# hpc4cmb/flacarray

Measured on AMD Instinct MI355X. Metric: Msamples/s encode+decode, 4096ch x 1Msamp int32, higher is better.
Workload: dtype int32

## Files before the change

### flacarray_amd/csrc/encode_fused.hpp

```cpp
#pragma once
#include "encode_kernels.hpp"
#include "quantize_kernels.hpp"

namespace fa {

constexpr int kFSmpWords = 65 * 32;
#ifndef FA_F_SCANW
#define FA_F_SCANW 4
#endif
#ifndef FA_F_RING
#define FA_F_RING 1024
#endif
constexpr int kFRingWords = FA_F_RING;
constexpr int kFRingMask = kFRingWords - 1;
constexpr int kFRingBlocks = kFRingWords / 64;
constexpr int kFRowBlocks = 12;
static_assert(kFRingBlocks - kFRowBlocks - 1 >= 1, "the ring must hold the longest row and a partial block beside what waits to be flushed");
constexpr int kFWaveWords = kFSmpWords + kFRingWords + 4 + 16;
constexpr int kFWaves = 4;
constexpr int kFCrcSlice = 1024;
constexpr int kFCrcXpow = 520;
#ifndef FA_F_SLEEP
#define FA_F_SLEEP 8
#endif
#ifndef FA_F_WBATCH
#define FA_F_WBATCH 4
#endif
#ifndef FA_F_CEIL
#define FA_F_CEIL 1
#endif
#ifndef FA_F_BFLY_N
#define FA_F_BFLY_N 1
#endif
#ifndef FA_F_SHLEV
#define FA_F_SHLEV 1
#endif
#ifndef FA_F_SHLEV_MAXMLO
#define FA_F_SHLEV_MAXMLO 12
#endif
#ifndef FA_F_SHPOLL
#define FA_F_SHPOLL 256
#endif
#ifndef FA_F_SHSLEEP
#define FA_F_SHSLEEP 4
#endif
#ifndef FA_F_PARKN
#define FA_F_PARKN 32
#endif
#ifndef FA_F_PARKBLK
#define FA_F_PARKBLK 1
#endif
#ifndef FA_F_PARK
#define FA_F_PARK 1
#endif
#ifndef FA_F_WAVES
#define FA_F_WAVES 3
#endif
constexpr uint32_t kLbSpinLimit = 1u << 22;

struct FusedArgs {
    const int32_t* data;
    const float* f_offsets;
    const float* f_gains;
    int64_t n_stream, stream_size, nframes, total_frames;
    int32_t max_lpc_order, max_porder, precision, pmax_full;
    int32_t tail_bs;
    double escale_full;
    const float* win;
    const uint4* hdr;
    uint8_t* blob;
    int64_t capacity;
    int64_t hb;
    uint32_t* frame_bytes;
    int64_t* frame_abs;
    FrameInfo* info;
    uint32_t* ticket;
    uint32_t* size_pub;
    unsigned long long* off_pub;
    int64_t* total;
    int* err;
    const uint16_t* crc_tab;
    unsigned long long* stamps;
    int64_t* starts;
    int64_t* nbytes;
};

__device__ __forceinline__ int fsmp_unit(int c1, int u) { return 32 * c1 + 4 * (u ^ (c1 & 7)); }
__device__ __forceinline__ int fsmp_idx(int s) {
    const int c1 = (s >> 5) + 1;
    return fsmp_unit(c1, (s >> 2) & 7) + (s & 3);
}

__device__ __forceinline__ int lane_id_opaque() {
    int l;
    asm volatile("v_mbcnt_lo_u32_b32 %0, -1, 0\n\tv_mbcnt_hi_u32_b32 %0, -1, %0" : "=v"(l));
    return l;
}
__device__ __forceinline__ int rice_fold(int r) { return (int)(((uint32_t)r << 1) ^ (uint32_t)(r >> 31)); }
__device__ __forceinline__ int dpp_wave_shr1(int old, int v) { return __builtin_amdgcn_update_dpp(old, v, 0x138, 0xF, 0xF, false); }

__device__ __forceinline__ uint16_t crc16_mulmod(uint16_t a, uint16_t b) {
    uint32_t r = 0;
#pragma unroll
    for (int i = 15; i >= 0; --i) {
        r = (r << 1) ^ ((r & 0x8000u) ? 0x18005u : 0u);
        if ((b >> i) & 1) r ^= a;
    }
    return (uint16_t)r;
}

template <typename T>
__device__ __forceinline__ T lb_load(const T* p) { return __hip_atomic_load(p, __ATOMIC_RELAXED, __HIP_MEMORY_SCOPE_AGENT); }

struct SplitRiceSearch {
    int pred_order, pmax, lane;
    uint32_t TA, TB, S, n, pb, SC, best;
    int M, p, k, bpo, kb;
    bool slot;
    __device__ __forceinline__ void start(uint32_t ta, uint32_t tb, int pred_order_, int pmax_, int lane_) {
        pred_order = pred_order_; pmax = pmax_; lane = lane_;
        TA = wave_incl_scan_u32(ta);
        TB = wave_incl_scan_u32(tb);
    }
    __device__ __forceinline__ void gather() {
        M = (2 << pmax) - 1;
        const int Lp = M - lane;
        slot = (Lp >= 1);
        const int po = slot ? (31 - __clz(Lp)) : 0;
        p = lane - (M + 1 - (2 << po));
        const uint32_t psz = 4096u >> po;
        const int cpp = 128 >> po;
        const bool inB = (po > 0) && (p >= (1 << (po - 1)));
        const int ph = inB ? (p - (1 << (po - 1))) : p;
        int hi_l = (po == 0) ? 63 : ((ph + 1) * cpp - 1);
        int lo_l = (po == 0) ? -1 : (ph * cpp - 1);
        hi_l &= 63;
        const int lo_c = lo_l < 0 ? 0 : (lo_l & 63);
        const uint32_t ah = (uint32_t)__builtin_amdgcn_ds_bpermute(hi_l << 2, (int)TA);
        const uint32_t bh = (uint32_t)__builtin_amdgcn_ds_bpermute(hi_l << 2, (int)TB);
        const uint32_t al = (uint32_t)__builtin_amdgcn_ds_bpermute(lo_c << 2, (int)TA);
        const uint32_t bl = (uint32_t)__builtin_amdgcn_ds_bpermute(lo_c << 2, (int)TB);
        uint32_t s;
        if (po == 0) s = ah + bh;
        else s = (inB ? bh : ah) - ((lo_l >= 0) ? (inB ? bl : al) : 0u);
        S = slot ? s : 0u;
        n = psz - ((p == 0) ? (uint32_t)pred_order : 0u);
        n = slot ? n : 1u;
    }
    __device__ __forceinline__ void params() {
        const uint32_t fpd = 0x40000u / n;
        const uint32_t m1 = S - 1;
        const uint32_t v = (__umulhi(m1, fpd) << 14) | ((m1 * fpd) >> 18);
        k = (S < 2 || v == 0) ? 0 : (32 - __clz((int)v));
        const uint32_t rest = (k != 0) ? (S >> ((k - 1) & 31)) : (S << 1);
        pb = 4u + (uint32_t)(1 + k) * n + rest - (n >> 1);
        pb = slot ? pb : 0u;
    }
    __device__ __forceinline__ void totals() {
        SC = wave_incl_scan_u32(pb);
        best = 0xffffffffu;
        bpo = 0;
        kb = 0;
    }
    __device__ __forceinline__ void order(int o) {
        const bool valid = (o <= pmax);
        const int base = valid ? (M + 1 - (2 << o)) : 0;
        const int end = valid ? (base + (1 << o) - 1) : 0;
        const uint32_t hi = (uint32_t)__builtin_amdgcn_readlane((int)SC, end);
        const uint32_t lo = (uint32_t)__builtin_amdgcn_readlane((int)SC, base > 0 ? base - 1 : 0);
        const uint32_t bits = hi - (base > 0 ? lo : 0u) + 6u;
        const int kg = __builtin_amdgcn_ds_bpermute(((base + lane) & 63) << 2, k);
        const bool take = valid && (bits < best);
        best = take ? bits : best;
        bpo = take ? o : bpo;
        kb = take ? kg : kb;
    }
};

__device__ __forceinline__ uint64_t split_rice_search_slow(uint64_t ta, uint64_t tb, int pred_order, int pmax, int lane, int* best_po,
                                                           int* kbest) {
    const uint64_t TA = wave_incl_scan_u64(ta), TB = wave_incl_scan_u64(tb);
    uint64_t best = 0;
    bool have = false;
    int bpo = 0, kb = 0;
    for (int po = pmax; po >= 0; --po) {
        const int nparts = 1 << po;
        const uint32_t psz = 4096u >> po;
        const int cpp = 128 >> po;
        const int p = lane & (nparts - 1);
        const bool inB = (po > 0) && (p >= (nparts >> 1));
        const int ph = inB ? (p - (nparts >> 1)) : p;
        const int hi_l = (po == 0) ? 63 : (((ph + 1) * cpp - 1) & 63);
        const int lo_l = (po == 0) ? -1 : (ph * cpp - 1);
        const int lo_c = lo_l < 0 ? 0 : (lo_l & 63);
        const uint64_t ah = gather_u64(TA, hi_l), bh = gather_u64(TB, hi_l), al = gather_u64(TA, lo_c), bl = gather_u64(TB, lo_c);
        uint64_t S;
        if (po == 0) S = ah + bh;
        else S = (inB ? bh : ah) - ((lo_l >= 0) ? (inB ? bl : al) : 0);
        uint64_t pb = 0;
        int k = 0;
        if (lane < nparts) {
            const uint32_t n = psz - ((lane == 0) ? (uint32_t)pred_order : 0u);
            k = rice_param(S, n);
// ... 142 lines not shown
                for (int o = 0; o < MLO; ++o) {
                    const double b = mbv[o];
                    if (o < usable && b < bestb) { bestb = b; bi = o; }
                }
            }
            wlo = bi + 1;
        }
        if (fbps <= 17) {
            const int limp = 32 - fbps - ilog2_u64((uint64_t)wlo);
            if (wprec > limp) wprec = limp;
        }
        wsh = 0;
#pragma unroll
        for (int j = 0; j < MLO; ++j) wq[j] = 0;
        wok = 0;
        if (wprec >= 2) wok = (quantize_coefs_t<MLO>(coef + (wlo - 1) * MLO, wlo, wprec, wq, &wsh) == 0) ? 1 : 0;
    };
    auto shlev_announce = [&](bool cand, int fbps, const double* ac) __attribute__((always_inline)) {
        const int ln = lane_id_opaque();
        if (ln == 0) {
            if (cand) {
#pragma unroll
                for (int j = 0; j <= MLO; ++j) lev_in[wave][j] = ac[j];
            }
            lev_bps[wave] = cand ? fbps : -1;
        }
        lds_fence();
        uint32_t before = 0;
        if (ln == 0) before = __hip_atomic_fetch_add(&lev_cnt, 1u, __ATOMIC_RELAXED, __HIP_MEMORY_SCOPE_WORKGROUP);
        lds_fence();
        if ((uint32_t)__builtin_amdgcn_readfirstlane((int)before) != (uint32_t)(kFWaves - 1)) return;
        const int fr = ln >> 4, sub = ln & 15;
        const int fbps_w = lev_bps[fr];
        double acw[MLO + 1];
#pragma unroll
        for (int j = 0; j <= MLO; ++j) acw[j] = lev_in[fr][j];
        if (fbps_w < 0) {
            acw[0] = 1.0;
#pragma unroll
            for (int j = 1; j <= MLO; ++j) acw[j] = 0.0;
        }
        int wok, wlo, wprec, wsh;
        int32_t wq[MLO];
        lpc_solve(std::integral_constant<int, 16>{}, acw, fbps_w, scr + 256 * fr, sub, wok, wlo, wprec, wsh, wq);
        if (sub == 0) {
            lev_out[fr][0] = wok; lev_out[fr][1] = wlo; lev_out[fr][2] = wprec; lev_out[fr][3] = wsh;
#pragma unroll
            for (int j = 0; j < MLO; ++j) lev_out[fr][4 + j] = wq[j];
        }
        lds_fence();
        if (sub == 0) __hip_atomic_store(&lev_rdy[fr], 1u, __ATOMIC_RELAXED, __HIP_MEMORY_SCOPE_WORKGROUP);
        lds_fence();
    };
    if constexpr (SHLEV) {
        bool mine = g < a.total_frames;
        if (mine && a.tail_bs != kMaxBlock) mine = ((uint32_t)g % (uint32_t)a.nframes) != (uint32_t)(a.nframes - 1);
        if (__builtin_expect(!mine, 0)) {
            shlev_announce(false, 0, nullptr);
            return;
        }
    }
    if (g >= a.total_frames) return;

    const int64_t s = (int64_t)((uint32_t)g / (uint32_t)a.nframes);
    const int64_t f = g - s * a.nframes;
    if (f == a.nframes - 1 && a.tail_bs != kMaxBlock) return;
    const int32_t* src = a.data + (s * a.stream_size + f * (int64_t)bs);
    float q_off = 0.0f, q_gain = 0.0f;
    if constexpr (F32IN) { q_off = a.f_offsets[s]; q_gain = a.f_gains[s]; }
    auto load_row = [&](int j) __attribute__((always_inline)) {
        const int4 v = reinterpret_cast<const int4*>(src)[64 * j + lane];
        if constexpr (F32IN)
            return make_int4(quantise_f32(__int_as_float(v.x), q_off, q_gain), quantise_f32(__int_as_float(v.y), q_off, q_gain),
                             quantise_f32(__int_as_float(v.z), q_off, q_gain), quantise_f32(__int_as_float(v.w), q_off, q_gain));
        else
            return v;
    };
    const float* win = a.win;
    const uint4 fhe = a.hdr[f];
    const uint32_t fh_bits = 32u + ((fhe.w >> 8) & 0xFFu) + ((fhe.w >> 16) & 0xFFu) + (fhe.w >> 24) + 8u;

#define FA_IMAGE_ADDRS                                                                  \
    const int ln_ = lane_id_opaque();                                                   \
    const int K = fsmp_unit(ln_ + 1, 0);                                                \
    const int rowbase = fsmp_unit((ln_ >> 3) + 1, ln_ & 7);                             \
    const int hist7 = fsmp_unit(ln_, 7), hist6 = fsmp_unit(ln_, 6), hist5 = fsmp_unit(ln_, 5); \
    (void)K; (void)rowbase; (void)hist7; (void)hist6; (void)hist5
    constexpr int tailA7 = 32 * 64 + 4 * (7 ^ (64 & 7)), tailA6 = 32 * 64 + 4 * (6 ^ (64 & 7)), tailA5 = 32 * 64 + 4 * (5 ^ (64 & 7));

    FA_STAMP_INIT;
#ifdef FA_TIMELINE
    const uint32_t tl_start_ = (uint32_t)__builtin_amdgcn_s_memrealtime();
#endif
    int4 Bv[8];
    uint32_t orv = 0;
    int mn, mx;
    {
        FA_IMAGE_ADDRS;
        int4 hi[8], lo[8];
#pragma unroll
        for (int j = 0; j < 8; ++j) hi[j] = load_row(8 + j);
#pragma unroll
        for (int j = 0; j < 8; ++j) lo[j] = load_row(j);
        if (lane < 32) smp[lane] = 0;
        mn = hi[0].x;
        mx = hi[0].x;
#pragma unroll
        for (int j = 0; j < 8; ++j) {
            orv |= (uint32_t)(hi[j].x | hi[j].y | hi[j].z | hi[j].w);
            mn = min(min(mn, hi[j].x), hi[j].y);
            mn = min(min(mn, hi[j].z), hi[j].w);
            mx = max(max(mx, hi[j].x), hi[j].y);
            mx = max(max(mx, hi[j].z), hi[j].w);
            *reinterpret_cast<int4*>(&smp[rowbase + 256 * j]) = hi[j];
        }
#pragma unroll
        for (int t = 0; t < 8; ++t) Bv[t] = *reinterpret_cast<const int4*>(&smp[K ^ (4 * t)]);
#pragma unroll
        for (int j = 0; j < 8; ++j) {
// ... 129 lines not shown
#pragma unroll
            for (int t = 0; t < 4; ++t) group(std::false_type{}, Bv[t], 0);
            fold();
#pragma unroll
            for (int t = 4; t < 8; ++t) group(std::false_type{}, Bv[t], 0);
            fold();
            tot0 = (double)a0; tot1 = (double)a1; tot2 = (double)a2; tot3 = (double)a3; tot4 = (double)a4;
        } else {
            FA_IMAGE_ADDRS;
            double p1, pe1, pe2, pe3;
            auto seed = [&](const int4& h) __attribute__((always_inline)) {
                p1 = (double)h.w;
                pe1 = (double)h.w - (double)h.z;
                const double e1b = (double)h.z - (double)h.y;
                pe2 = pe1 - e1b;
                const double e2b = e1b - ((double)h.y - (double)h.x);
                pe3 = pe2 - e2b;
            };
            auto group = [&](const int4& xv, int gi0) __attribute__((always_inline)) {
                const int xs[4] = {xv.x, xv.y, xv.z, xv.w};
#pragma unroll
                for (int e = 0; e < 4; ++e) {
                    const int gi = gi0 + e;
                    const double xd = (double)xs[e];
                    const double e1 = xd - p1;
                    const double e2 = e1 - pe1;
                    const double e3 = e2 - pe2;
                    const double e4 = e3 - pe3;
                    const double a0 = fa_fabs(xd);
                    const double a1 = (gi >= 1) ? fa_fabs(e1) : 0.0;
                    const double a2 = (gi >= 2) ? fa_fabs(e2) : 0.0;
                    const double a3 = (gi >= 3) ? fa_fabs(e3) : 0.0;
                    const double a4 = (gi >= 4) ? fa_fabs(e4) : 0.0;
                    tot0 += a0; tot1 += a1; tot2 += a2; tot3 += a3; tot4 += a4;
                    mx0 = __builtin_fmax(mx0, a0);
                    mx1 = __builtin_fmax(mx1, a1);
                    mx2 = __builtin_fmax(mx2, a2);
                    mx3 = __builtin_fmax(mx3, a3);
                    mx4 = __builtin_fmax(mx4, a4);
                    p1 = xd; pe1 = e1; pe2 = e2; pe3 = e3;
                }
            };
            seed(*reinterpret_cast<const int4*>(&smp[hist7]));
#pragma unroll 1
            for (int t = 0; t < 8; ++t) group(*reinterpret_cast<const int4*>(&smp[K ^ (4 * t)]), 32 * lane + 4 * t);
            dA0 = tot0; dA1 = tot1; dA2 = tot2; dA3 = tot3; dA4 = tot4;
            seed(hist_b(Bv[7], *reinterpret_cast<const int4*>(&smp[tailA7])));
#pragma unroll
            for (int t = 0; t < 8; ++t) group(Bv[t], 4096);
        }
        FA_STAMP(1);
        {
            double tsum[5] = {tot0, tot1, tot2, tot3, tot4};
            wave_sum_butterfly_n<5>(tsum);
            const double T0 = tsum[0], T1 = tsum[1], T2 = tsum[2], T3 = tsum[3], T4 = tsum[4];
            double M0 = 0.0, M1 = 0.0, M2 = 0.0, M3 = 0.0, M4 = 0.0;
            if (!narrow) {
                M0 = wave_max_f64(mx0); M1 = wave_max_f64(mx1); M2 = wave_max_f64(mx2); M3 = wave_max_f64(mx3);
                M4 = wave_max_f64(mx4);
            }
            const double lim = 2147483647.0;
            double smallest = 1.8446744073709552e19;
            if (M0 <= lim && T0 < smallest) { fo = 0; smallest = T0; }
            if (M1 <= lim && T1 < smallest) { fo = 1; smallest = T1; }
            if (M2 <= lim && T2 < smallest) { fo = 2; smallest = T2; }
            if (M3 <= lim && T3 < smallest) { fo = 3; smallest = T3; }
            if (M4 <= lim && T4 < smallest) { fo = 4; smallest = T4; }
        }
        if (narrow) {
            const uint64_t tA = (fo == 0) ? hA0 : (fo == 1) ? hA1 : (fo == 2) ? hA2 : (fo == 3) ? hA3 : hA4;
            const double tt = (fo == 0) ? tot0 : (fo == 1) ? tot1 : (fo == 2) ? tot2 : (fo == 3) ? tot3 : tot4;
            fixA = tA;
            fixB = (uint64_t)tt - tA;
        } else {
            const double tA = (fo == 0) ? dA0 : (fo == 1) ? dA1 : (fo == 2) ? dA2 : (fo == 3) ? dA3 : dA4;
            const double tt = (fo == 0) ? tot0 : (fo == 1) ? tot1 : (fo == 2) ? tot2 : (fo == 3) ? tot3 : tot4;
            fixA = (uint64_t)tA;
            fixB = (uint64_t)(tt - tA);
        }
        pmax_fix = pmax_for(fo < 0 ? 0 : fo);
        const bool small_fix = __all((fixA < (1u << 24)) && (fixB < (1u << 24)));
        win_small_f = small_fix;
        fuse_search = !SHLEV && fo >= 0 && pmax_fix <= 5 && a.max_lpc_order > 0 && small_fix;
        if (__builtin_expect(fo >= 0 && !fuse_search, SHLEV ? 1 : 0)) {
            uint64_t rb;
            if (pmax_fix <= 5 && small_fix) {
                SplitRiceSearch fs;
                fs.start((uint32_t)fixA, (uint32_t)fixB, fo, pmax_fix, lane);
                fs.gather(); fs.params(); fs.totals();
#pragma unroll
                for (int o = 5; o >= 0; --o) fs.order(o);
                po_fix = fs.bpo; k_fix = fs.kb; rb = fs.best;
            } else {
                rb = split_rice_search_slow(fixA, fixB, fo, pmax_fix, lane, &po_fix, &k_fix);
            }
            est_fix = 8 + (uint64_t)wasted + (uint64_t)fo * (uint64_t)bps + rb;
            apply_fixed();
        }
        FA_STAMP(2);
    };

    if (__builtin_expect(is_const, 0)) {
        type = 0;
    } else {
        if constexpr (!SHLEV) fixed_analysis();
        if (__builtin_expect(a.max_lpc_order > 0, 1)) {
            FA_IMAGE_ADDRS;
// ... 48 lines not shown
                    hist[j] = (double)hs[j] * (double)wh;
                }
#pragma unroll
                for (int tb = 0; tb < 8; tb += FA_F_WBATCH) {
                    WinV wv[FA_F_WBATCH];
#pragma unroll
                    for (int t = 0; t < FA_F_WBATCH; ++t) wv[t] = load_win(g0 + 4 * (tb + t));
#pragma unroll
                    for (int t = 0; t < FA_F_WBATCH; ++t) {
                        lag_group(*reinterpret_cast<const int4*>(&smp[K ^ (4 * (tb + t))]), wv[t]);
                        search_stage(tb + t);
                    }
                    __builtin_amdgcn_sched_barrier(0);
                }
            }
#if FA_F_PARK
            {
                uint32_t pin = 16u * (uint32_t)lane;
                asm volatile("" : "+v"(pin) : "v"(__double2loint(acc[MLO])));
                const int4* const pk = reinterpret_cast<const int4*>(reinterpret_cast<const char*>(ring) + pin);
#pragma unroll
                for (int t = 0; t < 4; ++t) Bv[4 + t] = pk[64 * t];
            }
#endif
            {
                const int g0 = 2048 + 32 * lane;
                const int4 h7 = hist_b(Bv[7], *reinterpret_cast<const int4*>(&smp[tailA7]));
                const int4 h6 = hist_b(Bv[6], *reinterpret_cast<const int4*>(&smp[tailA6]));
                int4 h5 = make_int4(0, 0, 0, 0);
                if constexpr (MLO > 8) h5 = hist_b(Bv[5], *reinterpret_cast<const int4*>(&smp[tailA5]));
                const int hs[12] = {h7.w, h7.z, h7.y, h7.x, h6.w, h6.z, h6.y, h6.x, h5.w, h5.z, h5.y, h5.x};
#pragma unroll
                for (int j = 0; j < MLO; ++j) hist[j] = (double)hs[j] * (double)win[g0 - 1 - j];
#pragma unroll
                for (int tb = 0; tb < 8; tb += FA_F_WBATCH) {
                    WinV wv[FA_F_WBATCH];
#pragma unroll
                    for (int t = 0; t < FA_F_WBATCH; ++t) wv[t] = load_win(g0 + 4 * (tb + t));
#pragma unroll
                    for (int t = 0; t < FA_F_WBATCH; ++t) {
                        lag_group(Bv[tb + t], wv[t]);
                        search_stage(8 + tb + t);
                    }
                    __builtin_amdgcn_sched_barrier(0);
                }
            }
            FA_STAMP(4);
            if (fuse_search) {
                po_fix = fs.bpo;
                k_fix = fs.kb;
                est_fix = 8 + (uint64_t)wasted + (uint64_t)fo * (uint64_t)bps + (uint64_t)fs.best;
                apply_fixed();
            }
#if FA_F_BFLY_N
#pragma unroll
            for (int j = 0; j <= MLO; ++j) autoc[j] = acc[j];
            wave_sum_butterfly_n<MLO + 1>(autoc);
#else
#pragma unroll
            for (int j = 0; j <= MLO; ++j) autoc[j] = wave_sum_butterfly(acc[j]);
#endif
            lpc_cand = (autoc[0] != 0.0);
        }
    }

    FA_STAMP(5);
    int ok = 0, lo = 0, prec = a.precision, sh = 0;
    int32_t qreg[MLO];
#pragma unroll
    for (int j = 0; j < MLO; ++j) qreg[j] = 0;
    if constexpr (SHLEV) {
        shlev_announce(lpc_cand, bps, autoc);
        FA_STAMP(6);
        if (!is_const) fixed_analysis();
        if (lpc_cand) {
#ifdef FA_STAMPS
            const unsigned long long tw0_ = fa_memtime();
#endif
            uint32_t up = 0, polls = 0;
            for (;;) {
                up = (uint32_t)__builtin_amdgcn_readfirstlane((int)__hip_atomic_load(&lev_rdy[wave], __ATOMIC_RELAXED, __HIP_MEMORY_SCOPE_WORKGROUP));
                if (up != 0 || ++polls > (uint32_t)FA_F_SHPOLL) break;
                __builtin_amdgcn_s_sleep(FA_F_SHSLEEP);
            }
            lds_fence();
#ifdef FA_STAMPS
            if (lane_id_opaque() == 0 && a.stamps && (blockIdx.x & 63) == 0) {
                atomicAdd(&a.stamps[17], fa_memtime() - tw0_);
                atomicAdd(&a.stamps[18], (unsigned long long)polls);
                atomicAdd(&a.stamps[19], up != 0 ? 0ULL : 1ULL);
                atomicAdd(&a.stamps[20], 1ULL);
            }
#endif
            if (__builtin_expect(up != 0, 1)) {
                ok = lev_out[wave][0]; lo = lev_out[wave][1]; prec = lev_out[wave][2]; sh = lev_out[wave][3];
#pragma unroll
                for (int j = 0; j < MLO; ++j) qreg[j] = lev_out[wave][4 + j];
            } else {
                lpc_solve(std::integral_constant<int, 64>{}, autoc, bps, scr, lane_id_opaque(), ok, lo, prec, sh, qreg);
            }
        }
    } else {
        if (lpc_cand) lpc_solve(std::integral_constant<int, 64>{}, autoc, bps, scr, lane, ok, lo, prec, sh, qreg);
        FA_STAMP(6);
    }
    ok = __builtin_amdgcn_readfirstlane(ok);
    lo = __builtin_amdgcn_readfirstlane(lo);
// ... 257 lines not shown
        }
        sub_bits = (uint32_t)exact;
    }
    if (type == 0) sub_bits = 8u + (uint32_t)wasted + (uint32_t)bps;
    if (type == 1) sub_bits = (uint32_t)verbatim_bits;
    const uint32_t total_bytes = ((fh_bits + sub_bits + 7u) >> 3) + 2u;
    const uint32_t L = total_bytes - 2u;

    FA_STAMP(9);
    const uint32_t F = (uint32_t)a.total_frames;
    const uint32_t gu = (uint32_t)g;
#ifdef FA_TIMELINE
    if (lane_w == 0 && a.info) {
        a.info[g].type = type;
        a.info[g].order = (type >= 2) ? order : 0;
        a.info[g].wasted = (int32_t)tl_start_;
        a.info[g].shift = (int32_t)(uint32_t)__builtin_amdgcn_s_memrealtime();
        __builtin_amdgcn_s_waitcnt(0);
    }
#endif
    if (lane_w == 0) {
        __hip_atomic_store(a.size_pub + gu, 0x80000000u | total_bytes, __ATOMIC_RELAXED, __HIP_MEMORY_SCOPE_AGENT);
        a.frame_bytes[g] = total_bytes;
    }
    (void)F;
#ifndef FA_TIMELINE
    if (lane_w == 0 && a.info) {
        FrameInfo fi;
        fi.type = type;
        fi.order = (type >= 2) ? order : 0;
        fi.porder = (type >= 2) ? porder : 0;
        fi.wasted = wasted;
        fi.shift = (type == 3) ? shift : 0;
        fi.precision = (type == 3) ? precision : 0;
        fi.nbytes = (int32_t)total_bytes;
        fi.blocksize = bs;
        a.info[g] = fi;
    }
#endif

#ifdef FA_F_ANALYSIS_ONLY
    if (lane_w == 0) a.frame_abs[g] = g * (int64_t)kSlotBytes + (s + 1) * a.hb;
    return;
#endif
    kpar[lane_w] = (uint8_t)kbest;
    for (int i = lane_w; i < kFRingWords; i += 64) ring[i] = 0;
    if (lane_w == 0) ring[kFRingWords] = 0;
    lds_fence();
    uint32_t pos = 0;
    uint32_t blocks_flushed = 0;
    uint8_t* dst = nullptr;
    bool dropped = false, have_dst = false;
    uint32_t crc_t = 0;

    auto put_bits = [&](uint32_t P, uint32_t val, uint32_t nb) __attribute__((always_inline)) {
        const uint32_t off = P & 31u;
        const uint64_t X = (uint64_t)val << (64u - nb - off);
        const uint32_t a0 = (P >> 3) & (uint32_t)(4 * kFRingWords - 4);
        atomicOr(reinterpret_cast<uint32_t*>(reinterpret_cast<char*>(ring) + a0), (uint32_t)(X >> 32));
        atomicOr(reinterpret_cast<uint32_t*>(reinterpret_cast<char*>(ring) + a0 + 4), (uint32_t)X);
    };
    auto put_code = [&](uint32_t P, uint32_t u, uint32_t shl) __attribute__((always_inline)) {
        const uint32_t vL = (u << shl) | 0x80000000u;
        uint32_t wi;
        asm("v_bfe_u32 %0, %1, 5, %2" : "=v"(wi) : "v"(P), "n"(__builtin_ctz((unsigned)kFRingWords)));
        uint32_t* const w = ring + wi;
        atomicOr(w, __builtin_amdgcn_alignbit(0u, vL, P));
        atomicOr(w + 1, __builtin_amdgcn_alignbit(vL, 0u, P));
    };
    unsigned long long off_word = 0;
    auto lb_issue = [&]() __attribute__((always_inline)) {
#ifndef FA_F_NOLB
        off_word = lb_load(a.off_pub + gu);
#endif
    };
    auto lb_resolve = [&]() __attribute__((always_inline)) {
        uint32_t spins = 0;
        bool fail = false;
#ifdef FA_TIMELINE
        const uint32_t tl_req_ = (uint32_t)__builtin_amdgcn_s_memrealtime();
#endif
#ifdef FA_F_NOLB
        off_word = (unsigned long long)(g * (int64_t)kSlotBytes + (s + 1) * a.hb);
#else
        while (off_word == 0) {
            __builtin_amdgcn_s_sleep(FA_F_SLEEP);
            if (++spins > kLbSpinLimit) { fail = true; break; }
            off_word = lb_load(a.off_pub + gu);
        }
#endif
#ifdef FA_TIMELINE
        if (lane_w == 0 && a.info) {
            a.info[g].precision = (int32_t)tl_req_;
            a.info[g].blocksize = (int32_t)(uint32_t)__builtin_amdgcn_s_memrealtime();
        }
#endif
#ifdef FA_STAMPS
        st_[3] += spins;
#endif
        const int64_t off = (int64_t)(((uint64_t)(uint32_t)__builtin_amdgcn_readfirstlane((int)(uint32_t)(off_word >> 32)) << 32) |
                                      (uint32_t)__builtin_amdgcn_readfirstlane((int)(uint32_t)off_word));
        fail = __builtin_amdgcn_readfirstlane((int)fail) != 0;
        if (fail || off < 0 || off + (int64_t)total_bytes > a.capacity) {
            if (lane_w == 0) atomicOr(a.err, fail ? 2 : 1);
            dropped = true;
        } else {
            dst = a.blob + off;
            if (lane_w == 0) a.frame_abs[g] = off;
        }
        have_dst = true;
    };
    auto crc_word = [&](uint32_t wv) __attribute__((always_inline)) {
        const uint32_t w = wv ^ (crc_t << 16);
        const uint32_t t0 = crc_s[w >> 24], t1 = crc_s[256 + ((w >> 16) & 255u)], t2 = crc_s[512 + ((w >> 8) & 255u)], t3 = crc_s[768 + (w & 255u)];
        uint32_t x01;
        asm("v_xor_b32 %0, %1, %2" : "=v"(x01) : "v"(t0), "v"(t1));
        asm("v_bitop3_b32 %0, %1, %2, %3 bitop3:0x96" : "=v"(crc_t) : "v"(x01), "v"(t2), "v"(t3));
    };
    uint32_t carry = 0;
    auto emit_word = [&](uint32_t m, uint32_t Q) __attribute__((always_inline)) {
        const uint32_t sh = (uint32_t)(reinterpret_cast<uintptr_t>(dst) & 3u);
        const uint32_t P = (uint32_t)dpp_wave_shr1((int)carry, (int)Q);
        carry = (uint32_t)__builtin_amdgcn_readlane((int)Q, 63);
        const uint32_t V = __builtin_amdgcn_alignbit(P, Q, 8u * sh);
        const int lo = (int)(4u * m) - (int)sh;
        if (lo >= 0 && (uint32_t)lo + 4u <= total_bytes) {
            *reinterpret_cast<uint32_t*>(dst + lo) = __builtin_bswap32(V);
        } else {
#pragma unroll
            for (int i = 0; i < 4; ++i) {
                const int b = lo + i;
                if (b >= 0 && (uint32_t)b < total_bytes) dst[b] = (uint8_t)(V >> (24 - 8 * i));
            }
        }
    };
    auto emit_block = [&](uint32_t blk, uint32_t Q) __attribute__((always_inline)) {
        const uint32_t sh = (uint32_t)(reinterpret_cast<uintptr_t>(dst) & 3u);
        const uint32_t P = (uint32_t)dpp_wave_shr1((int)carry, (int)Q);
        carry = (uint32_t)__builtin_amdgcn_readlane((int)Q, 63);
        const uint32_t V = __builtin_amdgcn_alignbit(P, Q, 8u * sh);
        *reinterpret_cast<uint32_t*>(dst - sh + 256u * blk + 4u * (uint32_t)lane_w) = __builtin_bswap32(V);
    };
#if FA_F_PARKBLK
    uint32_t park[FA_F_PARKN];
#endif
    uint32_t n_parked = 0;
    auto take_block = [&](uint32_t blk) __attribute__((always_inline)) {
        const uint32_t wi = (blk * 64 + lane_w) & kFRingMask;
        uint32_t wv = ring[wi];
        ring[wi] = 0;
        if (__builtin_expect((blk & (uint32_t)(kFRingBlocks - 1)) == 0, 0)) {
            if (lane_w == 0) { wv |= ring[kFRingWords]; ring[kFRingWords] = 0; }
        }
        return wv;
    };
    auto flush_blocks = [&](uint32_t row_bits, bool final_call) __attribute__((always_inline)) {
        const uint32_t done = (uint32_t)__builtin_amdgcn_readfirstlane((int)(pos >> 11));
        blocks_flushed = (uint32_t)__builtin_amdgcn_readfirstlane((int)blocks_flushed);
        const uint32_t hi_blk = (uint32_t)__builtin_amdgcn_readfirstlane((int)((pos + row_bits) >> 11));
        if (!final_call && hi_blk - blocks_flushed < (uint32_t)kFRingBlocks) return;
#ifdef FA_STAMPS
        const unsigned long long tq0_ = fa_memtime();
#endif
        if (!have_dst) {
#if FA_F_PARKBLK
            if (!final_call && off_word == 0) {
                off_word = lb_load(a.off_pub + gu);
                n_parked = (uint32_t)__builtin_amdgcn_readfirstlane((int)n_parked);
                while (blocks_flushed < done && n_parked < (uint32_t)FA_F_PARKN) {
                    const uint32_t wv = take_block(blocks_flushed);
                    crc_word(wv);
                    park[n_parked] = wv;
                    n_parked++;
                    blocks_flushed++;
                }
                if (hi_blk - blocks_flushed < (uint32_t)kFRingBlocks) {
#ifdef FA_STAMPS
                    st_[14] += fa_memtime() - tq0_;
#endif
                    return;
                }
            }
#endif
            lb_resolve();
        }
#ifdef FA_STAMPS
        st_[14] += fa_memtime() - tq0_;
#endif
#if FA_F_PARKBLK
        n_parked = (uint32_t)__builtin_amdgcn_readfirstlane((int)n_parked);
        if (__builtin_expect(n_parked != 0, 0)) {
            if (!dropped) {
                emit_word((uint32_t)lane_w, park[0]);
                for (uint32_t i = 1; i < n_parked; ++i) emit_block(i, park[i]);
            }
            n_parked = 0;
        }
#endif
        if (__builtin_expect(blocks_flushed == 0 && done > 0, 0)) {
            const uint32_t wv = take_block(0);
            crc_word(wv);
            if (!dropped) emit_word((uint32_t)lane_w, wv);
            blocks_flushed = 1;
// ... 332 lines not shown
```

### flacarray_amd/csrc/encode_kernels.hpp

```cpp
#pragma once
#include <hip/hip_runtime.h>
#include <stdint.h>

#include <type_traits>

#include "flac_math.hpp"

namespace fa {

#ifndef FA_UNIT_COMPACT

struct FrameInfo {
    int32_t type, order, porder, wasted, shift, precision, nbytes, blocksize;
};

struct EncodeArgs {
    const int32_t* data;
    int64_t n_stream;
    int64_t stream_size;
    int64_t nframes;
    int32_t B;
    int32_t tail_bs;
    int32_t max_lpc_order;
    int32_t max_porder;
// ... 96 lines not shown
constexpr int kDppXor2 = 0x4E;
constexpr int kDppHalfMirror = 0x141;
constexpr int kDppMirror = 0x140;
constexpr int kSwzXor16 = 0x401F;

template <int STEP>
__device__ __forceinline__ int xchg_i32(int v) {
    if constexpr (STEP == 0) return dpp_i32<kDppXor1>(v);
    else if constexpr (STEP == 1) return dpp_i32<kDppXor2>(v);
    else if constexpr (STEP == 2) return dpp_i32<kDppHalfMirror>(v);
    else if constexpr (STEP == 3) return dpp_i32<kDppMirror>(v);
    else return __builtin_amdgcn_ds_swizzle(v, kSwzXor16);
}
template <int STEP>
__device__ __forceinline__ double xchg_f64(double v) {
    const int lo = xchg_i32<STEP>(__double2loint(v)), hi = xchg_i32<STEP>(__double2hiint(v));
    return __hiloint2double(hi, lo);
}
template <int STEP>
__device__ __forceinline__ uint64_t xchg_u64(uint64_t v) {
    const uint32_t lo = (uint32_t)xchg_i32<STEP>((int)(uint32_t)v), hi = (uint32_t)xchg_i32<STEP>((int)(uint32_t)(v >> 32));
    return ((uint64_t)hi << 32) | lo;
}
__device__ __forceinline__ double readlane_f64(double v, int l) {
    return __hiloint2double(__builtin_amdgcn_readlane(__double2hiint(v), l), __builtin_amdgcn_readlane(__double2loint(v), l));
}
__device__ __forceinline__ uint64_t readlane_u64(uint64_t v, int l) {
    return ((uint64_t)(uint32_t)__builtin_amdgcn_readlane((int)(uint32_t)(v >> 32), l) << 32) |
           (uint32_t)__builtin_amdgcn_readlane((int)(uint32_t)v, l);
}

__device__ __forceinline__ double wave_sum_butterfly(double v) {
    v = v + xchg_f64<0>(v);
    v = v + xchg_f64<1>(v);
    v = v + xchg_f64<2>(v);
    v = v + xchg_f64<3>(v);
    v = v + xchg_f64<4>(v);
    return readlane_f64(v, 0) + readlane_f64(v, 32);
}
template <int N>
__device__ __forceinline__ void wave_sum_butterfly_n(double (&v)[N]) {
    double o[N];
#define FA_BF_STEP(S)                                          \
    _Pragma("unroll") for (int i = 0; i < N; ++i) o[i] = xchg_f64<S>(v[i]); \
    _Pragma("unroll") for (int i = 0; i < N; ++i) v[i] = v[i] + o[i];
    FA_BF_STEP(0)
    FA_BF_STEP(1)
    FA_BF_STEP(2)
    FA_BF_STEP(3)
    FA_BF_STEP(4)
#undef FA_BF_STEP
#pragma unroll
    for (int i = 0; i < N; ++i) v[i] = readlane_f64(v[i], 0) + readlane_f64(v[i], 32);
}
__device__ __forceinline__ double wave_max_f64(double v) {
    double o;
    o = xchg_f64<0>(v); v = (o > v) ? o : v;
    o = xchg_f64<1>(v); v = (o > v) ? o : v;
    o = xchg_f64<2>(v); v = (o > v) ? o : v;
    o = xchg_f64<3>(v); v = (o > v) ? o : v;
    o = xchg_f64<4>(v); v = (o > v) ? o : v;
    const double a = readlane_f64(v, 0), b = readlane_f64(v, 32);
    return (b > a) ? b : a;
}
__device__ __forceinline__ uint64_t wave_sum_u64(uint64_t v) {
    v += xchg_u64<0>(v);
    v += xchg_u64<1>(v);
    v += xchg_u64<2>(v);
    v += xchg_u64<3>(v);
    v += xchg_u64<4>(v);
    return readlane_u64(v, 0) + readlane_u64(v, 32);
}
__device__ __forceinline__ uint32_t wave_or_u32(uint32_t v) {
    v |= (uint32_t)xchg_i32<0>((int)v);
    v |= (uint32_t)xchg_i32<1>((int)v);
    v |= (uint32_t)xchg_i32<2>((int)v);
    v |= (uint32_t)xchg_i32<3>((int)v);
    v |= (uint32_t)xchg_i32<4>((int)v);
    return (uint32_t)__builtin_amdgcn_readlane((int)v, 0) | (uint32_t)__builtin_amdgcn_readlane((int)v, 32);
}
__device__ __forceinline__ int wave_min_i32(int v) {
    v = min(v, xchg_i32<0>(v));
    v = min(v, xchg_i32<1>(v));
    v = min(v, xchg_i32<2>(v));
    v = min(v, xchg_i32<3>(v));
    v = min(v, xchg_i32<4>(v));
    return min(__builtin_amdgcn_readlane(v, 0), __builtin_amdgcn_readlane(v, 32));
}
__device__ __forceinline__ int wave_max_i32(int v) {
    v = max(v, xchg_i32<0>(v));
    v = max(v, xchg_i32<1>(v));
    v = max(v, xchg_i32<2>(v));
    v = max(v, xchg_i32<3>(v));
    v = max(v, xchg_i32<4>(v));
    return max(__builtin_amdgcn_readlane(v, 0), __builtin_amdgcn_readlane(v, 32));
}
__device__ __forceinline__ uint32_t wave_incl_scan_u32(uint32_t v) {
    v += (uint32_t)__builtin_amdgcn_update_dpp(0, (int)v, 0x111, 0xF, 0xF, true);
    v += (uint32_t)__builtin_amdgcn_update_dpp(0, (int)v, 0x112, 0xF, 0xF, true);
    v += (uint32_t)__builtin_amdgcn_update_dpp(0, (int)v, 0x114, 0xF, 0xF, true);
    v += (uint32_t)__builtin_amdgcn_update_dpp(0, (int)v, 0x118, 0xF, 0xF, true);
    v += (uint32_t)__builtin_amdgcn_update_dpp(0, (int)v, 0x142, 0xA, 0xF, false);
    v += (uint32_t)__builtin_amdgcn_update_dpp(0, (int)v, 0x143, 0xC, 0xF, false);
    return v;
}

// ... 1391 lines not shown
```

### flacarray_amd/csrc/flac_math.hpp

```cpp
#pragma once
#include <stdint.h>

#if defined(__HIPCC__)
#define FA_HD __host__ __device__ __forceinline__
#else
#define FA_HD inline
#endif

#if defined(FA_UNIT_FUSED) || defined(FA_UNIT_PLACED)
#define FA_GLOBAL static
#else
#define FA_GLOBAL
#endif

namespace fa {

constexpr int kMaxBlock = 4096;
constexpr int kChunk = 64;
constexpr int kRow = 256;
constexpr int kRowCapBits = 12288;
constexpr int kRiceLimit = 31;
constexpr int kMaxLpcOrder = 12;
constexpr int kSlotBytes = 16640;

struct LevelParams {
    int blocksize;
    int max_lpc_order;
    int max_porder;
    int qlp_precision;
};

FA_HD LevelParams level_params(uint32_t level) {
    const int lpc[9] = {0, 0, 0, 6, 8, 8, 8, 12, 12};
    const int po[9] = {3, 3, 3, 4, 4, 5, 6, 6, 6};
    LevelParams p;
    p.blocksize = (level <= 2) ? 1152 : 4096;
    p.max_lpc_order = lpc[level];
    p.max_porder = po[level];
    p.qlp_precision = (p.blocksize <= 384) ? 13 : (p.blocksize <= 1152 ? 14 : 15);
    return p;
}

FA_HD uint64_t dbits(double x) {
    union { double d; uint64_t u; } c;
    c.d = x;
    return c.u;
}
FA_HD double bitsd(uint64_t u) {
    union { double d; uint64_t u; } c;
    c.u = u;
    return c.d;
}

FA_HD int ilog2_u64(uint64_t v) {
#if defined(__HIP_DEVICE_COMPILE__)
    return 63 - __clzll((long long)v);
#else
    return 63 - __builtin_clzll(v);
#endif
}

FA_HD double det_log2(double x) {
    uint64_t b = dbits(x);
    int e = (int)((b >> 52) & 0x7ff) - 1023;
    double m = bitsd((b & 0x000fffffffffffffULL) | 0x3ff0000000000000ULL);
    if (m > 1.4142135623730951) { m = m * 0.5; e += 1; }
    double s = (m - 1.0) / (m + 1.0);
    double z = s * s;
    double p = 1.0 / 21.0;
    p = p * z + 1.0 / 19.0;
    p = p * z + 1.0 / 17.0;
    p = p * z + 1.0 / 15.0;
    p = p * z + 1.0 / 13.0;
    p = p * z + 1.0 / 11.0;
    p = p * z + 1.0 / 9.0;
    p = p * z + 1.0 / 7.0;
    p = p * z + 1.0 / 5.0;
    p = p * z + 1.0 / 3.0;
    p = p * z + 1.0;
    return (double)e + (2.8853900817779268 * s) * p;
}

FA_HD double fa_floor(double x) {
#if defined(__HIP_DEVICE_COMPILE__)
    return __builtin_floor(x);
#else
    return __builtin_floor(x);
#endif
}
FA_HD double fa_ceil(double x) { return __builtin_ceil(x); }
FA_HD double fa_fabs(double x) { return __builtin_fabs(x); }

template <int MLO>
FA_HD int levinson(const double* autoc, int max_order, float* coef, double* err_out) {
    double lpc[MLO];
    double err = autoc[0];
#pragma unroll
    for (int i = 0; i < MLO; ++i) {
        if (i < max_order) {
            double r = -autoc[i + 1];
#pragma unroll
            for (int j = 0; j < MLO; ++j)
                if (j < i) r = r - lpc[j] * autoc[i - j];
            r = r / err;
// ... 166 lines not shown
```

### flacarray_amd/csrc/flacarray_hip.hip

```cpp
#include <hip/hip_runtime.h>

#include <cmath>
#include <cstdio>
#include <cstdlib>
#include <cstring>
#include <algorithm>
#include <atomic>
#include <condition_variable>
#include <functional>
#include <map>
#include <memory>
#include <mutex>
#include <new>
#include <thread>
#include <vector>

#include <sys/mman.h>
#include <time.h>
#include <unistd.h>

#include "../../include/flacarray_hip.h"
#include "decode_kernels.hpp"
#ifndef FA_SPLIT_UNITS
#define FA_HAVE_K5_LAUNCHERS 1
// ... 1146 lines not shown
    if (slots_forced()) return nch == 2 ? fa_encode_workspace_bytes_i64(n_stream, stream_size, level) : fa_encode_workspace_bytes(n_stream, stream_size, level);
    PlacedPlan pp;
    if (make_placed_plan(n_stream, stream_size, level, nch, &pp) != FA_ERROR_NONE) return -1;
    int64_t need = (int64_t)pp.total;
    if (nch == 1 && fused_geometry(n_stream, stream_size, level)) {
        FusedPlan pl;
        make_fused_plan(n_stream, stream_size, level, &pl);
        need = std::max<int64_t>(need, (int64_t)pl.total);
    }
    return need;
}
int64_t fa_encode_single_pass_workspace_bytes(int64_t n_stream, int64_t stream_size, uint32_t level) {
    return single_pass_workspace_for(n_stream, stream_size, level, 1);
}
int64_t fa_encode_single_pass_workspace_bytes_i64(int64_t n_stream, int64_t stream_size, uint32_t level) {
    return single_pass_workspace_for(n_stream, stream_size, level, 2);
}

static int fused_encode_run(const void* d_data, bool f32, const float* d_quanta, float* d_offsets, float* d_gains, int64_t n_stream,
                            int64_t stream_size, uint32_t level, void* d_workspace, int64_t workspace_bytes, unsigned char* d_bytes,
                            int64_t capacity_bytes, int64_t* d_starts, int64_t* d_nbytes, int64_t* h_total_bytes, int32_t* d_info,
                            void* stream) {
    FA_API_LOCK;
    FusedPlan pl;
    make_fused_plan(n_stream, stream_size, level, &pl);
    if (!d_workspace || workspace_bytes < (int64_t)pl.total) return FA_ERROR_ALLOC;
    if (!d_bytes || capacity_bytes < n_stream * pl.hb + 64) return FA_ERROR_ALLOC;
    hipStream_t st = reinterpret_cast<hipStream_t>(stream);
    char* ws = reinterpret_cast<char*>(d_workspace);
    prof_begin(3, st);
    int* d_nanflag = reinterpret_cast<int*>(ws + pl.off_ticket + 12);
    FA_HIP_TRY(hipMemsetAsync(ws + pl.off_zero, 0, pl.zero_bytes, st));
    if (f32) {
        const int64_t cps = (stream_size + kRangeChunk - 1) / kRangeChunk;
        void* pp = nullptr;
        int rcp = get_scratch(10, (size_t)n_stream * (size_t)cps * 8 + 256, &pp);
        if (rcp) return rcp;
        float* pmin = reinterpret_cast<float*>(pp);
        float* pmax = pmin + n_stream * cps;
        prof_begin(5, st);
        hipLaunchKernelGGL(float32_range_kernel, dim3((unsigned)(n_stream * cps)), dim3(256), 0, st, reinterpret_cast<const float*>(d_data),
                           stream_size, cps, pmin, pmax, d_nanflag);
        hipLaunchKernelGGL(float32_params_kernel, dim3((unsigned)((n_stream + 255) / 256)), dim3(256), 0, st, pmin, pmax, n_stream, cps,
                           d_quanta, d_offsets, d_gains);
        prof_end(5, st);
    }
    FusedArgs a;
    std::memset(&a, 0, sizeof a);
    a.data = reinterpret_cast<const int32_t*>(d_data); a.f_offsets = d_offsets; a.f_gains = d_gains; a.n_stream = n_stream; a.stream_size = stream_size; a.nframes = pl.nf; a.total_frames = pl.F;
    a.max_lpc_order = pl.P.max_lpc_order; a.max_porder = pl.P.max_porder; a.precision = pl.P.qlp_precision;
    a.pmax_full = max_porder_for(kMaxBlock, a.max_porder, 0);
    a.escale_full = 0.5 / (double)kMaxBlock;
    a.tail_bs = pl.tail_bs;
    const bool tails = (pl.tail_bs != kMaxBlock);
    int rc = get_window(kMaxBlock, &a.win);
    if (rc) return rc;
    rc = get_crc_tab_fused(&a.crc_tab);
    if (rc) return rc;
    {
        void* dp = nullptr;
        rc = get_scratch(9, (size_t)pl.nf * sizeof(uint4) + 256, &dp);
        if (rc) return rc;
        if (ds_->c_nf != pl.nf || ds_->c_B != kMaxBlock || ds_->c_tail != pl.tail_bs || ds_->c_nch != 1 || ds_->c_dp != dp ||
            ds_->c_epoch != ds_->scratch_epoch) {
            ds_->h_hdr.resize((size_t)pl.nf);
            for (int64_t f = 0; f < pl.nf; ++f)
                ds_->h_hdr[(size_t)f] = frame_header_entry((uint64_t)f, (f == pl.nf - 1) ? pl.tail_bs : kMaxBlock, 1);
            FA_HIP_TRY(hipMemcpyAsync(dp, ds_->h_hdr.data(), (size_t)pl.nf * sizeof(uint4), hipMemcpyHostToDevice, st));
            FA_HIP_TRY(hipStreamSynchronize(st));
            ds_->c_nf = pl.nf; ds_->c_B = kMaxBlock; ds_->c_tail = pl.tail_bs; ds_->c_nch = 1; ds_->c_dp = dp; ds_->c_epoch = ds_->scratch_epoch;
        }
        a.hdr = reinterpret_cast<const uint4*>(dp);
    }
    a.blob = d_bytes; a.capacity = capacity_bytes; a.hb = pl.hb;
    a.frame_bytes = reinterpret_cast<uint32_t*>(ws + pl.off_fbytes);
    a.frame_abs = reinterpret_cast<int64_t*>(ws + pl.off_fabs);
    a.info = reinterpret_cast<FrameInfo*>(d_info);
    a.size_pub = reinterpret_cast<uint32_t*>(ws + pl.off_size);
    a.off_pub = reinterpret_cast<unsigned long long*>(ws + pl.off_off);
    a.total = reinterpret_cast<int64_t*>(ws + pl.off_ticket + 16);
    a.ticket = reinterpret_cast<uint32_t*>(ws + pl.off_ticket);
    a.err = reinterpret_cast<int*>(ws + pl.off_ticket + 8);
#ifdef FA_STAMPS
    {
        void* sp = nullptr;
        if (get_scratch(6, 512, &sp) == 0) {
            if (!ds_->stamps_zeroed) { (void)hipMemset(sp, 0, 512); ds_->stamps_zeroed = true; }
            a.stamps = reinterpret_cast<unsigned long long*>(sp);
        }
    }
#endif
    if (tails) {
        EncodeArgs t;
        std::memset(&t, 0, sizeof t);
        t.data = a.data; t.n_stream = n_stream; t.stream_size = stream_size; t.nframes = pl.nf; t.B = kMaxBlock; t.tail_bs = pl.tail_bs;
        t.max_lpc_order = a.max_lpc_order; t.max_porder = a.max_porder; t.precision = a.precision;
        t.win = a.win;
        rc = get_window(pl.tail_bs, &t.win_tail);
        if (rc) return rc;
        t.slots = reinterpret_cast<uint8_t*>(ws + pl.off_tslots); t.slot_stride = kSlotBytes;
        t.frame_bytes = a.frame_bytes; t.info = a.info; t.hdr = a.hdr;
        t.pmax_full = a.pmax_full; t.pmax_tail = max_porder_for(pl.tail_bs, a.max_porder, 0);
        t.escale_full = a.escale_full; t.escale_tail = 0.5 / (double)pl.tail_bs;
        t.tail_only = 1;
#ifdef FA_DEV_MINIMAL
        launch_encode<8, 1>(t, n_stream, st);
// ... 1666 lines not shown
```

Measured before the change: 211,000.

## Replace divisions with reciprocals, transpose wave reductions, and streamline ring flush addressing

Adds four independent micro-optimisations to the fused encoder, each enabled by default through its own macro. Integer divisions become a reciprocal-based quotient for the Rice parameter and a host-computed magic multiplier for the stream/frame split. The butterfly wave sums are replaced by transposed DPP pair reductions that fold several values at once. The output flush now uses a byte-perm with a precomputed selector, a rotated DPP carry instead of readlane, and scalar-base addressing for ring and block stores. The aim is fewer VALU, SALU and cross-lane instructions in the hot per-frame path, at the cost of more inline asm and the risk of subtle correctness problems in the byte-order and carry handling.

New measurement: 213,900 (median of 2 runs). About the same (+1.4%).

```diff
diff --git a/flacarray_amd/csrc/encode_fused.hpp b/flacarray_amd/csrc/encode_fused.hpp
--- a/flacarray_amd/csrc/encode_fused.hpp
+++ b/flacarray_amd/csrc/encode_fused.hpp
@@ -53,6 +53,15 @@
 #ifndef FA_F_PARK
 #define FA_F_PARK 1
 #endif
+#ifndef FA_F_FLUSH2
+#define FA_F_FLUSH2 1
+#endif
+#ifndef FA_F_TSUM
+#define FA_F_TSUM 1
+#endif
+#ifndef FA_F_NODIV
+#define FA_F_NODIV 1
+#endif
 #ifndef FA_F_WAVES
 #define FA_F_WAVES 3
 #endif
@@ -65,6 +74,7 @@
     int64_t n_stream, stream_size, nframes, total_frames;
     int32_t max_lpc_order, max_porder, precision, pmax_full;
     int32_t tail_bs;
+    uint32_t nf_magic;
     double escale_full;
     const float* win;
     const uint4* hdr;
@@ -98,6 +108,7 @@
 }
 __device__ __forceinline__ int rice_fold(int r) { return (int)(((uint32_t)r << 1) ^ (uint32_t)(r >> 31)); }
 __device__ __forceinline__ int dpp_wave_shr1(int old, int v) { return __builtin_amdgcn_update_dpp(old, v, 0x138, 0xF, 0xF, false); }
+__device__ __forceinline__ int dpp_wave_ror1(int v) { return __builtin_amdgcn_update_dpp(0, v, 0x13C, 0xF, 0xF, true); }
 
 __device__ __forceinline__ uint16_t crc16_mulmod(uint16_t a, uint16_t b) {
     uint32_t r = 0;
@@ -148,7 +159,11 @@
         n = slot ? n : 1u;
     }
     __device__ __forceinline__ void params() {
+#if FA_F_NODIV
+        const uint32_t fpd = fpd18_div(n);
+#else
         const uint32_t fpd = 0x40000u / n;
+#endif
         const uint32_t m1 = S - 1;
         const uint32_t v = (__umulhi(m1, fpd) << 14) | ((m1 * fpd) >> 18);
         k = (S < 2 || v == 0) ? 0 : (32 - __clz((int)v));
@@ -397,19 +412,23 @@
         if (sub == 0) __hip_atomic_store(&lev_rdy[fr], 1u, __ATOMIC_RELAXED, __HIP_MEMORY_SCOPE_WORKGROUP);
         lds_fence();
     };
-    if constexpr (SHLEV) {
-        bool mine = g < a.total_frames;
-        if (mine && a.tail_bs != kMaxBlock) mine = ((uint32_t)g % (uint32_t)a.nframes) != (uint32_t)(a.nframes - 1);
-        if (__builtin_expect(!mine, 0)) {
-            shlev_announce(false, 0, nullptr);
-            return;
-        }
-    }
-    if (g >= a.total_frames) return;
-
-    const int64_t s = (int64_t)((uint32_t)g / (uint32_t)a.nframes);
-    const int64_t f = g - s * a.nframes;
-    if (f == a.nframes - 1 && a.tail_bs != kMaxBlock) return;
+    bool mine = g < a.total_frames;
+    uint32_t s_u = 0, f_u = 0;
+    if (mine) {
+#if FA_F_NODIV
+        if (__builtin_expect(a.nf_magic != 0u, 1)) s_u = __umulhi((uint32_t)g, a.nf_magic);
+        else
+#endif
+            s_u = (uint32_t)g / (uint32_t)a.nframes;
+        f_u = (uint32_t)g - s_u * (uint32_t)a.nframes;
+        if (a.tail_bs != kMaxBlock && f_u == (uint32_t)(a.nframes - 1)) mine = false;
+    }
+    if (__builtin_expect(!mine, 0)) {
+        if constexpr (SHLEV) shlev_announce(false, 0, nullptr);
+        return;
+    }
+    const int64_t s = (int64_t)s_u;
+    const int64_t f = (int64_t)f_u;
     const int32_t* src = a.data + (s * a.stream_size + f * (int64_t)bs);
     float q_off = 0.0f, q_gain = 0.0f;
     if constexpr (F32IN) { q_off = a.f_offsets[s]; q_gain = a.f_gains[s]; }
@@ -645,7 +664,11 @@
         FA_STAMP(1);
         {
             double tsum[5] = {tot0, tot1, tot2, tot3, tot4};
+#if FA_F_TSUM
+            wave_sum_transposed_n<5>(tsum);
+#else
             wave_sum_butterfly_n<5>(tsum);
+#endif
             const double T0 = tsum[0], T1 = tsum[1], T2 = tsum[2], T3 = tsum[3], T4 = tsum[4];
             double M0 = 0.0, M1 = 0.0, M2 = 0.0, M3 = 0.0, M4 = 0.0;
             if (!narrow) {
@@ -800,7 +823,11 @@
                 est_fix = 8 + (uint64_t)wasted + (uint64_t)fo * (uint64_t)bps + (uint64_t)fs.best;
                 apply_fixed();
             }
-#if FA_F_BFLY_N
+#if FA_F_TSUM
+#pragma unroll
+            for (int j = 0; j <= MLO; ++j) autoc[j] = acc[j];
+            wave_sum_transposed_n<MLO + 1>(autoc);
+#elif FA_F_BFLY_N
 #pragma unroll
             for (int j = 0; j <= MLO; ++j) autoc[j] = acc[j];
             wave_sum_butterfly_n<MLO + 1>(autoc);
@@ -1164,6 +1191,12 @@
     uint8_t* dst = nullptr;
     bool dropped = false, have_dst = false;
     uint32_t crc_t = 0;
+#if FA_F_FLUSH2
+    uint32_t* const ring_lane = ring + lane_w;
+    uint32_t lane4_w = 4u * (uint32_t)lane_w;
+    uint32_t rotq = 0;
+    uint32_t bsel = 0x00010203u;
+#endif
 
     auto put_bits = [&](uint32_t P, uint32_t val, uint32_t nb) __attribute__((always_inline)) {
         const uint32_t off = P & 31u;
@@ -1218,6 +1251,9 @@
             dropped = true;
         } else {
             dst = a.blob + off;
+#if FA_F_FLUSH2
+            bsel = 0x00010203u + 0x01010101u * (uint32_t)(reinterpret_cast<uintptr_t>(dst) & 3u);
+#endif
             if (lane_w == 0) a.frame_abs[g] = off;
         }
         have_dst = true;
@@ -1229,38 +1265,63 @@
         asm("v_xor_b32 %0, %1, %2" : "=v"(x01) : "v"(t0), "v"(t1));
         asm("v_bitop3_b32 %0, %1, %2, %3 bitop3:0x96" : "=v"(crc_t) : "v"(x01), "v"(t2), "v"(t3));
     };
+#if FA_F_FLUSH2
+    auto aligned_dword = [&](uint32_t Q) __attribute__((always_inline)) {
+        const uint32_t P = (uint32_t)dpp_wave_shr1((int)rotq, (int)Q);
+        const uint32_t W = __builtin_amdgcn_perm(P, Q, bsel);
+        uint32_t Qr = Q;
+        asm("" : "+v"(Qr) : "v"(W));
+        rotq = (uint32_t)dpp_wave_ror1((int)Qr);
+        return W;
+    };
+#else
     uint32_t carry = 0;
-    auto emit_word = [&](uint32_t m, uint32_t Q) __attribute__((always_inline)) {
+    auto aligned_dword = [&](uint32_t Q) __attribute__((always_inline)) {
         const uint32_t sh = (uint32_t)(reinterpret_cast<uintptr_t>(dst) & 3u);
         const uint32_t P = (uint32_t)dpp_wave_shr1((int)carry, (int)Q);
         carry = (uint32_t)__builtin_amdgcn_readlane((int)Q, 63);
-        const uint32_t V = __builtin_amdgcn_alignbit(P, Q, 8u * sh);
+        return __builtin_bswap32(__builtin_amdgcn_alignbit(P, Q, 8u * sh));
+    };
+#endif
+    auto emit_word = [&](uint32_t m, uint32_t Q) __attribute__((always_inline)) {
+        const uint32_t sh = (uint32_t)(reinterpret_cast<uintptr_t>(dst) & 3u);
+        const uint32_t W = aligned_dword(Q);
         const int lo = (int)(4u * m) - (int)sh;
         if (lo >= 0 && (uint32_t)lo + 4u <= total_bytes) {
-            *reinterpret_cast<uint32_t*>(dst + lo) = __builtin_bswap32(V);
+            *reinterpret_cast<uint32_t*>(dst + lo) = W;
         } else {
 #pragma unroll
             for (int i = 0; i < 4; ++i) {
                 const int b = lo + i;
-                if (b >= 0 && (uint32_t)b < total_bytes) dst[b] = (uint8_t)(V >> (24 - 8 * i));
+                if (b >= 0 && (uint32_t)b < total_bytes) dst[b] = (uint8_t)(W >> (8 * i));
             }
         }
     };
     auto emit_block = [&](uint32_t blk, uint32_t Q) __attribute__((always_inline)) {
         const uint32_t sh = (uint32_t)(reinterpret_cast<uintptr_t>(dst) & 3u);
-        const uint32_t P = (uint32_t)dpp_wave_shr1((int)carry, (int)Q);
-        carry = (uint32_t)__builtin_amdgcn_readlane((int)Q, 63);
-        const uint32_t V = __builtin_amdgcn_alignbit(P, Q, 8u * sh);
-        *reinterpret_cast<uint32_t*>(dst - sh + 256u * blk + 4u * (uint32_t)lane_w) = __builtin_bswap32(V);
+        const uint32_t W = aligned_dword(Q);
+#if FA_F_FLUSH2
+        uint64_t bp = reinterpret_cast<uint64_t>(dst - sh + 256u * (uint32_t)__builtin_amdgcn_readfirstlane((int)blk));
+        asm volatile("" : "+s"(bp), "+v"(lane4_w));
+        *reinterpret_cast<__attribute__((address_space(1))) uint32_t*>(bp + (uint64_t)lane4_w) = W;
+#else
+        *reinterpret_cast<uint32_t*>(dst - sh + 256u * blk + 4u * (uint32_t)lane_w) = W;
+#endif
     };
 #if FA_F_PARKBLK
     uint32_t park[FA_F_PARKN];
 #endif
     uint32_t n_parked = 0;
     auto take_block = [&](uint32_t blk) __attribute__((always_inline)) {
+#if FA_F_FLUSH2
+        uint32_t* const wp = ring_lane + 64u * ((uint32_t)__builtin_amdgcn_readfirstlane((int)blk) & (uint32_t)(kFRingBlocks - 1));
+        uint32_t wv = *wp;
+        *wp = 0;
+#else
         const uint32_t wi = (blk * 64 + lane_w) & kFRingMask;
         uint32_t wv = ring[wi];
         ring[wi] = 0;
+#endif
         if (__builtin_expect((blk & (uint32_t)(kFRingBlocks - 1)) == 0, 0)) {
             if (lane_w == 0) { wv |= ring[kFRingWords]; ring[kFRingWords] = 0; }
         }
diff --git a/flacarray_amd/csrc/encode_kernels.hpp b/flacarray_amd/csrc/encode_kernels.hpp
--- a/flacarray_amd/csrc/encode_kernels.hpp
+++ b/flacarray_amd/csrc/encode_kernels.hpp
@@ -172,6 +172,73 @@
 #undef FA_BF_STEP
 #pragma unroll
     for (int i = 0; i < N; ++i) v[i] = readlane_f64(v[i], 0) + readlane_f64(v[i], 32);
+}
+#define FA_TSUM_PAIR(NAME, FWD, BACK, MASK)                                                                                   \
+    __device__ __forceinline__ double NAME(double a, double b) {                                                              \
+        const int alo = __double2loint(a), ahi = __double2hiint(a), blo = __double2loint(b), bhi = __double2hiint(b);        \
+        int ulo, uhi, wlo, whi;                                                                                               \
+        asm("s_mov_b32 vcc_lo, " MASK "\n\ts_mov_b32 vcc_hi, " MASK "\n\t"                                                    \
+            "v_cndmask_b32_dpp %0, %4, %6, vcc " FWD " row_mask:0xf bank_mask:0xf bound_ctrl:1\n\t"                            \
+            "v_cndmask_b32_dpp %1, %5, %7, vcc " FWD " row_mask:0xf bank_mask:0xf bound_ctrl:1\n\t"                            \
+            "s_not_b64 vcc, vcc\n\t"                                                                                          \
+            "v_cndmask_b32_dpp %2, %6, %4, vcc " BACK " row_mask:0xf bank_mask:0xf bound_ctrl:1\n\t"                           \
+            "v_cndmask_b32_dpp %3, %7, %5, vcc " BACK " row_mask:0xf bank_mask:0xf bound_ctrl:1"                                \
+            : "=&v"(ulo), "=&v"(uhi), "=&v"(wlo), "=&v"(whi)                                                                  \
+            : "v"(alo), "v"(ahi), "v"(blo), "v"(bhi)                                                                          \
+            : "vcc", "scc");                                                                                                  \
+        return __hiloint2double(uhi, ulo) + __hiloint2double(whi, wlo);                                                       \
+    }
+FA_TSUM_PAIR(tsum_pair0, "quad_perm:[1,0,3,2]", "quad_perm:[1,0,3,2]", "0xaaaaaaaa")
+FA_TSUM_PAIR(tsum_pair1, "quad_perm:[2,3,0,1]", "quad_perm:[2,3,0,1]", "0xcccccccc")
+FA_TSUM_PAIR(tsum_pair2, "row_shl:4", "row_shr:4", "0xf0f0f0f0")
+FA_TSUM_PAIR(tsum_pair3, "row_ror:8", "row_ror:8", "0xff00ff00")
+#undef FA_TSUM_PAIR
+constexpr int kDppRowRor8 = 0x128;
+template <int S, int M>
+__device__ __forceinline__ void tsum_step(const double (&in)[M], double (&out)[(M + 1) / 2]) {
+#pragma unroll
+    for (int i = 0; i < M / 2; ++i) {
+        if constexpr (S == 0) out[i] = tsum_pair0(in[2 * i], in[2 * i + 1]);
+        else if constexpr (S == 1) out[i] = tsum_pair1(in[2 * i], in[2 * i + 1]);
+        else if constexpr (S == 2) out[i] = tsum_pair2(in[2 * i], in[2 * i + 1]);
+        else out[i] = tsum_pair3(in[2 * i], in[2 * i + 1]);
+    }
+    if constexpr ((M & 1) != 0) {
+        const double x = in[M - 1];
+        if constexpr (S == 0 || S == 1) out[M / 2] = x + xchg_f64<S>(x);
+        else if constexpr (S == 2) out[M / 2] = tsum_pair2(x, x);
+        else out[M / 2] = x + __hiloint2double(dpp_i32<kDppRowRor8>(__double2hiint(x)), dpp_i32<kDppRowRor8>(__double2loint(x)));
+    }
+}
+constexpr int tsum_lane(int N, int j) {
+    int pos = j, M = N, lane = 0;
+    for (int s = 0; s < 4; ++s) {
+        const bool single = ((M & 1) != 0) && pos == M - 1;
+        if (!single) lane |= (pos & 1) << s;
+        pos >>= 1;
+        M = (M + 1) / 2;
+    }
+    return lane;
+}
+template <int N, int J = 0>
+__device__ __forceinline__ void tsum_collect(double t, double (&v)[N]) {
+    if constexpr (J < N) {
+        v[J] = readlane_f64(t, tsum_lane(N, J)) + readlane_f64(t, tsum_lane(N, J) + 32);
+        tsum_collect<N, J + 1>(t, v);
+    }
+}
+template <int N>
+__device__ __forceinline__ void wave_sum_transposed_n(double (&v)[N]) {
+    static_assert(N >= 1 && N <= 16, "four halving steps must leave one value");
+    constexpr int M1 = (N + 1) / 2, M2 = (M1 + 1) / 2, M3 = (M2 + 1) / 2, M4 = (M3 + 1) / 2;
+    static_assert(M4 == 1, "");
+    double l1[M1], l2[M2], l3[M3], l4[M4];
+    tsum_step<0, N>(v, l1);
+    tsum_step<1, M1>(l1, l2);
+    tsum_step<2, M2>(l2, l3);
+    tsum_step<3, M3>(l3, l4);
+    const double t = l4[0] + xchg_f64<4>(l4[0]);
+    tsum_collect<N>(t, v);
 }
 __device__ __forceinline__ double wave_max_f64(double v) {
     double o;
diff --git a/flacarray_amd/csrc/flac_math.hpp b/flacarray_amd/csrc/flac_math.hpp
--- a/flacarray_amd/csrc/flac_math.hpp
+++ b/flacarray_amd/csrc/flac_math.hpp
@@ -50,6 +50,24 @@
     union { double d; uint64_t u; } c;
     c.u = u;
     return c.d;
+}
+
+FA_HD uint32_t fpd18_div(uint32_t n) {
+#if defined(__HIP_DEVICE_COMPILE__)
+    const float r = __builtin_amdgcn_rcpf((float)n);
+    const uint32_t q = (uint32_t)(262144.0f * r);
+    const uint32_t rem = 262144u - __umul24(q, n);
+#else
+    const float r = 1.0f / (float)n;
+    const uint32_t q = (uint32_t)(262144.0f * r);
+    const uint32_t rem = 262144u - q * n;
+#endif
+    return q + (rem >= n ? 1u : 0u);
+}
+
+FA_HD uint32_t nframes_magic(uint64_t d, uint64_t total) {
+    if (d < 2 || total > (1ULL << 32) / d) return 0u;
+    return (uint32_t)((1ULL << 32) / d + 1ULL);
 }
 
 FA_HD int ilog2_u64(uint64_t v) {
diff --git a/flacarray_amd/csrc/flacarray_hip.hip b/flacarray_amd/csrc/flacarray_hip.hip
--- a/flacarray_amd/csrc/flacarray_hip.hip
+++ b/flacarray_amd/csrc/flacarray_hip.hip
@@ -1222,6 +1222,7 @@
     a.pmax_full = max_porder_for(kMaxBlock, a.max_porder, 0);
     a.escale_full = 0.5 / (double)kMaxBlock;
     a.tail_bs = pl.tail_bs;
+    a.nf_magic = nframes_magic((uint64_t)pl.nf, (uint64_t)pl.F);
     const bool tails = (pl.tail_bs != kMaxBlock);
     int rc = get_window(kMaxBlock, &a.win);
     if (rc) return rc;
```
